# Derek-TH-Wang/OpenRoboRL

Hardware: AMD Instinct MI355X
Metric: env steps/sec at N parallel robots (higher is better)
Workload: dtype f32

## Files before the change

openroborl_amd/csrc/orr_env_kernels.h:

```cpp
#pragma once
#if defined(ORR_PHASE_TIMERS) && !defined(ORR_WAVE_TIMELINE)
#define ORR_WAVE_TIMELINE 1
#endif
#ifndef ORR_TU_MAIN
#undef ORR_PHASE_TIMERS
#endif
#include <hip/hip_runtime.h>
#include <type_traits>
#include <math.h>
#include <stdint.h>
#include <stdio.h>
#include <stdlib.h>
#include <string.h>

#include "orr_device.h"

#ifdef ORR_PHASE_TIMERS
__device__ long long g_phase_cycles[orr::kPhaseSlots];
__device__ long long g_wave_phases[2048 * 40];
#define PT_INIT() do { if (threadIdx.x == 0) { for (int i_ = 0; i_ < orr::kPhaseSlots; i_++) S.pt_acc[i_] = 0; S.pt_last = clock64(); } } while (0)
#define PT(k) do { if (threadIdx.x == 0) { const long long t_ = clock64(); S.pt_acc[k] += t_ - S.pt_last; S.pt_last = clock64(); } } while (0)
#define PT_FLUSH() do { if (threadIdx.x == 0 && blockIdx.x == gridDim.x / 2) for (int i_ = 0; i_ < orr::kPhaseSlots; i_++) atomicAdd((unsigned long long*)&g_phase_cycles[i_], (unsigned long long)S.pt_acc[i_]); \
                        if (threadIdx.x == 0 && blockIdx.x < 2048) for (int i_ = 0; i_ < orr::kPhaseSlots; i_++) g_wave_phases[blockIdx.x * 40 + i_] = S.pt_acc[i_]; } while (0)
#else
// ... 16 lines not shown
#define ORR_DUAL_COUNT(k, cond) do { const unsigned long long b_ = __ballot(cond), act_ = __ballot(1); \
    if (b_ && (int)(threadIdx.x & 63u) == __ffsll((long long)act_) - 1) atomicAdd(&g_dual_contact[k], (unsigned long long)__popcll(b_)); } while (0)
#else
#define ORR_DUAL_COUNT(k, cond)
#endif

using namespace orr;

#define O(name) ORR_OFF_##name

#include "orr_robot_io.h"
#include "orr_physics.h"
#include "orr_task.h"

#define ORR_PROLOGUE()                                                                   \
  __shared__ Shared Sarr[kRPW];                                                          \
  const int wtid = (int)threadIdx.x;                                                     \
  const int wave_id = (int)blockIdx.x;                                                   \
  const int sub = wtid / kLanes, lane = wtid % kLanes;                                   \
  Shared& S = Sarr[sub];                                                                 \
  float* obs = S.ph.end.obs;                                                             \
  const int robot_raw = wave_id * kRPW + sub;                                            \
  const bool in_range = robot_raw < P.cfg.num_robots;                                    \
  const int robot = in_range ? robot_raw : 0;  \
  float* rec = P.state + (size_t)robot * ORR_STATE_STRIDE

template <bool CLIPS = false, bool NOISE = false>
__global__ __launch_bounds__(64) void orr_reset_kernel(KParams P, const uint8_t* mask, float* obs_out, const float* uniforms) {
  ORR_PROLOGUE();
  const bool valid = in_range && !(mask && !mask[robot]);
  load_robot(P, rec, S, lane);
  const long long total = P.counters[ORR_CNT_TOTAL_STEP_COUNT];
  const ResetConst RC = load_reset_const(P, S, lane);
  reset_robot<CLIPS, NOISE>(P, rec, S, lane, valid, total, obs, RC, uniforms ? uniforms + (size_t)robot * 28 : nullptr);
  WSYNC();
  store_robot(rec, S, lane, valid);
  if (valid)
    for (int i = lane; i < ORR_OFFEND_ANCHOR_VALID - ORR_OFF_ANCHOR + 1; i += kLanes) rec[O(ANCHOR) + i] = 0.0f;
  if (obs_out && valid)
    for (int i = lane; i < ORR_OBS_DIM; i += kLanes) obs_out[(size_t)robot * ORR_OBS_DIM + i] = obs[i];
}

#ifndef ORR_WAVES_PER_EU
#define ORR_WAVES_PER_EU 1
#endif
template <int MODE, int WPE = ORR_WAVES_PER_EU, bool ANCHOR = false, bool CLIPS = false, bool NOISE = false>
__global__ __launch_bounds__(64) __attribute__((amdgpu_waves_per_eu(WPE, WPE))) void orr_step_kernel(KParams P, const float* actions, float* obs_out, float* reward_out,
                                                      uint8_t* done_out, int nsub, ReplayArgs RP) {
  constexpr bool TERMS = (MODE & kModeTerms) != 0;
  static_assert(!TERMS || (MODE & 3) != 1, "the debug physics computes no reward");
  constexpr bool CONTACTS = (MODE & kModeContacts) != 0;
  static_assert(!CONTACTS || (MODE & 3) != 2, "the parity replay replaces the physics by recorded states: it has no impulses");
  constexpr bool ACT = (MODE & kModeActuator) != 0;
  static_assert(!ACT || (MODE & 3) != 1, "the debug physics takes its torques as given");
  static_assert(!ACT || TERMS, "the actuator variants are supersets: instantiated with the reward terms only");
  ORR_PROLOGUE();
  const bool valid = in_range;
  const orr_config& c = P.cfg;
  PT_INIT();
  WT_INIT();
  const long long total_snapshot = P.counters[ORR_CNT_TOTAL_STEP_COUNT];
  load_robot(P, rec, S, lane);
  bool terms_bound = true, contacts_bound = true, act_bound = false;
  if constexpr (ACT) {
    terms_bound = P.tab->terms != nullptr;
    contacts_bound = P.tab->contact_out != nullptr;
    act_bound = P.tab->act_out != nullptr;
  }
// ... 186 lines not shown
  bool switched = false;
  if constexpr (CLIPS) {
    if (t >= (double)clip_change) {
      typedef const int __attribute__((address_space(1)))* gip;
      typedef const float __attribute__((address_space(1)))* gfp;
      const int type = geti(S, O(ROBOT_TYPE));
      const int set_n = ((gip)&P.tab->clip_set_n[0])[type];
      const float sw_min = ((gfp)&P.tab->clip_switch[type][0])[0], sw_max = ((gfp)&P.tab->clip_switch[type][0])[1];
      if (set_n > 1 && sw_max < INFINITY) {
        float u4[4];
        philox_block(c.seed, (uint32_t)geti(S, O(ROBOT_INDEX)), (uint32_t)geti(S, O(EPISODE_IDX)), 8u + (uint32_t)geti(S, O(EP_STEP)), u4);
        const uint32_t m = (uint32_t)(u4[0] * 16777216.0f);
        const int k = (int)((m * (uint32_t)set_n) >> 24);
        const int id = ((gip)&P.tab->clip_set[type][0])[k];
        clip_change = clip_change_time(t, sw_min, sw_max, u4[1]);
        WSYNC();
        if (lane == 0) seti(S, O(CLIP_ID), id);
        const unsigned int* cg = reinterpret_cast<const unsigned int*>(&P.tab->clip[id]);
        unsigned int* cl = reinterpret_cast<unsigned int*>(&S.clip);
        if (lane < (int)(sizeof(DevClip) / 4)) cl[lane] = cg[lane];
        WSYNC();
        if (lane == 0) {
          S.s[O(TIME_OFFSET)] = u4[2] * (float)clip.dur_d;
          if (valid) rec[O(CLIP_CHANGE_TIME)] = clip_change;
        }
        WSYNC();
        t = motion_time(P, S);
        switched = true;
      }
    }
  }
  const double step_dt = clip.sim_dt_d * c.action_repeat;
  double tl = t;
  {
    const int k = lane - 1;
    const int steps = (k & 2) ? ((k & 1) ? c.tar_frame_steps[3] : c.tar_frame_steps[2]) : ((k & 1) ? c.tar_frame_steps[1] : c.tar_frame_steps[0]);
    if (lane >= 1 && lane <= 4) tl = t + steps * step_dt;
  }
  PoseLoads PL;
  sample_poses_issue(P, S, lane, tl, PL);
  typedef float __attribute__((address_space(1)))* gterm;
  float term = 0.0f, term_sum = 0.0f;
  if constexpr (TERMS) {
    if (lane < 5 && terms_bound) term_sum = ((gterm)P.tab->term_sums)[(size_t)robot * 5 + lane];
  }
  float c_ep = 0.0f;
  if constexpr (CONTACTS) {
    if (lane < 8 && contacts_bound) c_ep = ((gcontact)P.tab->contact_ep)[(size_t)robot * 8 + lane];
  }
  float a_ep = 0.0f;
  if constexpr (ACT && (MODE & 3) == 0) {
    if (lane < 4 && act_bound) a_ep = ((gact)P.tab->act_ep)[(size_t)robot * 4 + lane];
  }
  float rew;
  if constexpr (TERMS) {
    float tk[5];
    rew = calc_reward<true>(P, S, lane, (MODE & 3) == 2 ? RP.eff + (size_t)robot * 48 : nullptr, tk);
    term = lane == 0 ? tk[0] : (lane == 1 ? tk[1] : (lane == 2 ? tk[2] : (lane == 3 ? tk[3] : tk[4])));
  } else {
    rew = calc_reward(P, S, lane, (MODE & 3) == 2 ? RP.eff + (size_t)robot * 48 : nullptr);
  }
  sample_poses_finish(P, S, lane, tl, true, PL);
  {
    const float ph = clip_phase(clip, t_phase);
    if (lane == 0) {
      bool sync_pos = (c.flags & ORR_FLAG_CYCLE_SYNC) && ph < S.s[O(PREV_PHASE)];
      if constexpr (CLIPS) {
        if (switched) {
          q_about_z(task_heading(S, &S.s[O(QUAT)]) - task_heading(S, &S.ph.end.pose[0][3]), &S.s[O(ORIGIN_ROT)]);
          sync_pos = true;
        }
      }
      if (sync_pos) {
        float pr[3];
        qrot(&S.ph.end.pose[0][0], &S.s[O(ORIGIN_ROT)], pr);
        S.s[O(ORIGIN_POS)] = S.s[O(POS)] - pr[0];
        S.s[O(ORIGIN_POS) + 1] = S.s[O(POS) + 1] - pr[1];
        S.s[O(ORIGIN_POS) + 2] = 0.0f;
      }
      S.s[O(PREV_PHASE)] = ph;
      float v[3];
      qrot(&S.ph.end.vel[0], &S.s[O(ORIGIN_ROT)], v); S.ph.end.vel[0] = v[0]; S.ph.end.vel[1] = v[1]; S.ph.end.vel[2] = v[2];
      qrot(&S.ph.end.vel[3], &S.s[O(ORIGIN_ROT)], v); S.ph.end.vel[3] = v[0]; S.ph.end.vel[4] = v[1]; S.ph.end.vel[5] = v[2];
    }
    WSYNC();
    apply_origin(S, lane, 5);
    for (int i = lane; i < 19; i += kLanes) S.s[O(REF_POSE) + i] = S.ph.end.pose[0][i];
    for (int i = lane; i < 18; i += kLanes) S.s[O(REF_VEL) + i] = S.ph.end.vel[i];
    WSYNC();
  }
  PT(12);
  int reason = 0;
  unsigned long long log_slot = __builtin_nondeterministic_value(log_slot);
  uint32_t noise_i = 0u;
  {
    const float* rp = &S.s[O(REF_POSE)];
    float pe = 0.0f, qc[4], dq[4];
#pragma unroll
    for (int k = 0; k < 3; k++) { float d = rp[k] - S.s[O(POS) + k]; pe += d * d; }
    qconj(&S.s[O(QUAT)], qc);
    qmul(rp + 3, qc, dq);
    const float ang = q_norm_angle(dq);
    if (geti(S, O(STEP_COUNTER)) > 0 && fall) reason |= ORR_DONE_CONTACT_FALL;
    if (pe > c.dist_fail_threshold * c.dist_fail_threshold) reason |= ORR_DONE_ROOT_POS;
    if (fabsf(ang) > c.rot_fail_threshold) reason |= ORR_DONE_ROOT_ROT;
    if (!(clip.flags & ORR_CLIP_WRAP) && t >= clip.dur_d) reason |= ORR_DONE_MOTION_OVER;
    bool bad = false;
    for (int i = lane; i < 37; i += kLanes) bad = bad || !(fabsf(S.s[O(POS) + i]) < 1e30f);
    if (((__ballot(bad) >> (sub * kLanes)) & ((1ull << (kLanes - 1)) * 2ull - 1ull)) != 0ull || S.s[kHead - 1] != 0.0f) reason |= ORR_DONE_NAN;
    if (!(fabsf(rew) < 1e30f)) reason |= ORR_DONE_NAN;
    if (reason & ORR_DONE_NAN) rew = 0.0f;
    const int ep_step = geti(S, O(EP_STEP)) + 1;
    if constexpr (TERMS) {
      if (reason & ORR_DONE_NAN) term = 0.0f;
      term_sum = (ep_step == 1 ? 0.0f : term_sum) + term;
    }
    if constexpr (CONTACTS) {
      if (reason & ORR_DONE_NAN) c_sum = c_max = 0.0f;
      const float nsum = __shfl(c_sum, sub * kLanes + 3 * ((lane & 7) >> 1));
      const float add = nsum > 0.0f ? ((lane & 1) ? nsum : 1.0f) : 0.0f;
      c_ep = (ep_step == 1 ? 0.0f : c_ep) + add;
    }
    if constexpr (ACT) {
      a_w *= c.sim_dt;
      if (reason & ORR_DONE_NAN) a_s1 = a_pk = a_s2 = a_w = 0.0f;
      if constexpr ((MODE & 3) == 0) {
        const bool motor = lane < 12;
        const float w_all = row_sum16(motor ? a_w : 0.0f), s2_all = row_sum16(motor ? a_s2 : 0.0f), pk_all = row_max16(motor ? a_pk : 0.0f);
        const float sat_all = row_max16(motor && !(reason & ORR_DONE_NAN) && a_pk == a_lim ? 1.0f : 0.0f);
        const float old = ep_step == 1 ? 0.0f : a_ep;
        a_ep = lane == 2 ? fmaxf(old, pk_all) : old + (lane == 0 ? w_all : (lane == 1 ? s2_all : sat_all));
      }
    }
    if constexpr (NOISE) noise_i = (uint32_t)ep_step;
    if (ep_step >= geti(S, O(MAX_EP_STEPS))) reason |= ORR_DONE_TIME_LIMIT;
    if (lane == 0 && valid && reason != 0) log_slot = atomicAdd((unsigned long long*)&P.counters[ORR_CNT_EPISODES], 1ull);
    WSYNC();
    if (lane == 0) {
      seti(S, O(EP_STEP), ep_step);
      seti(S, O(DONE_REASON), reason);
      S.s[O(EP_RETURN)] += rew;
    }
  }
  if (lane < 12) obs[lane] = S.s[O(IMU_HIST) + lane];
  for (int i = lane; i < 36; i += kLanes) { obs[12 + i] = S.s[O(LASTACT_HIST) + i]; obs[48 + i] = S.s[O(MOTORANG_HIST) + i]; }
  target_obs<NOISE>(P, rec, S, lane, obs + ORR_PROPRIO_DIM, (uint32_t)geti(S, O(EPISODE_IDX)), noise_i);
  if (valid && lane == 0) {
    reward_out[robot] = rew;
    done_out[robot] = reason != 0;
  }
  if constexpr (TERMS) {
    if (valid && lane < 5 && terms_bound) {
      ((gterm)P.tab->terms)[(size_t)robot * 5 + lane] = term;
      ((gterm)P.tab->term_sums)[(size_t)robot * 5 + lane] = term_sum;
    }
  }
  if constexpr (CONTACTS) {
    store_contacts();
    if (valid && lane < 8 && contacts_bound) ((gcontact)P.tab->contact_ep)[(size_t)robot * 8 + lane] = c_ep;
  }
  if constexpr (ACT) {
    if (valid && lane < 12 && act_bound) {
      typedef f4 __attribute__((address_space(1)))* gact4;
      ((gact4)reinterpret_cast<f4*>(P.tab->act_out))[(size_t)robot * 12 + lane] = f4{a_s1, a_pk, a_s2, a_w};
    }
    if constexpr ((MODE & 3) == 0) {
      if (valid && lane < 4 && act_bound) ((gact)P.tab->act_ep)[(size_t)robot * 4 + lane] = a_ep;
    }
  }
  PT(13);
  if (reason != 0) {
    float log_ret = 0.0f, log_len = 0.0f;
    int log_clip = 0;
    const bool logs = lane == 0 && valid;
    const unsigned long long slot = log_slot;
    if (lane == 0) {
      log_ret = S.s[O(EP_RETURN)]; log_len = (float)geti(S, O(EP_STEP));
      if constexpr (CLIPS) log_clip = geti(S, O(CLIP_ID));
      S.s[O(LAST_EP_RETURN)] = log_ret;
      seti(S, O(LAST_EP_LEN), geti(S, O(EP_STEP)));
    }
    WSYNC();
    if (c.flags & ORR_FLAG_AUTO_RESET) {
      PT(31);
      reset_robot<CLIPS, NOISE>(P, rec, S, lane, valid, total_snapshot, obs, RC);
      if constexpr (ANCHOR) AS = AnchorState{{0.0f, 0.0f, 0.0f}, {0.0f, 0.0f, 0.0f}, 0};
    }
    if (logs && P.ep_log) {
      if (slot < (unsigned long long)P.ep_log_cap) {
        P.ep_log[2 * slot] = log_ret;
        P.ep_log[2 * slot + 1] = log_len;
        if constexpr (CLIPS) {
          int* const clip_log = P.tab->clip_log;
          if (clip_log) clip_log[slot] = log_clip;
        }
      } else {
        atomicAdd((unsigned long long*)&P.counters[ORR_CNT_EPLOG_DROPPED], 1ull);
      }
    }
    if constexpr (TERMS) {
      const int src = sub * kLanes;
      const unsigned long long tslot = ((unsigned long long)(unsigned)__shfl((int)(slot >> 32), src) << 32) | (unsigned)__shfl((int)slot, src);
      gterm const term_log = (gterm)P.tab->term_log;
      if (valid && lane < 5 && P.ep_log && term_log && tslot < (unsigned long long)P.ep_log_cap) term_log[tslot * 5 + lane] = term_sum;
    }
    if constexpr (CONTACTS) {
      const int src = sub * kLanes;
      const unsigned long long cslot = ((unsigned long long)(unsigned)__shfl((int)(slot >> 32), src) << 32) | (unsigned)__shfl((int)slot, src);
      gcontact const contact_log = (gcontact)P.tab->contact_log;
      if (valid && lane < 8 && P.ep_log && contact_log && cslot < (unsigned long long)P.ep_log_cap) contact_log[cslot * 8 + lane] = c_ep;
    }
    if constexpr (ACT && (MODE & 3) == 0) {
      const int src = sub * kLanes;
      const unsigned long long aslot = ((unsigned long long)(unsigned)__shfl((int)(slot >> 32), src) << 32) | (unsigned)__shfl((int)slot, src);
      gact const act_log = (gact)P.tab->act_log;
      if (valid && lane < 4 && P.ep_log && act_log && aslot < (unsigned long long)P.ep_log_cap) act_log[aslot * 4 + lane] = a_ep;
    }
  }
  WSYNC();
  PT(14);
  store_robot(rec, S, lane, valid);
  store_anchor();
  if (valid) {
    typedef f4 __attribute__((address_space(1))) * g4ptr;
    static_assert(ORR_OBS_DIM % 4 == 0, "16-byte pieces");
    const g4ptr od = (g4ptr)reinterpret_cast<f4*>(obs_out + (size_t)robot * ORR_OBS_DIM);
    const f4* os = reinterpret_cast<const f4*>(obs);
#pragma unroll
    for (int k = 0; k < (ORR_OBS_DIM / 4 + kLanes - 1) / kLanes; k++) { const int q = lane + k * kLanes; if (q < ORR_OBS_DIM / 4) od[q] = os[q]; }
  }
  PT(15);
  PT_FLUSH();
  const unsigned long long fin_mask = __ballot(valid && lane == 0 && reason != 0), val_mask = __ballot(valid && lane == 0);
  if (wtid == 0) {
    const unsigned long long add = ((unsigned long long)__popcll(fin_mask) << 32) | (unsigned long long)__popcll(val_mask);
    const unsigned long long now = atomicAdd((unsigned long long*)&P.counters[ORR_CNT_TICKET], add) + add;
    if ((unsigned int)now == (unsigned int)P.cfg.num_robots) {
      atomicAdd((unsigned long long*)&P.counters[ORR_CNT_TOTAL_STEP_COUNT], now >> 32);
      atomicAdd((unsigned long long*)&P.counters[ORR_CNT_TOTAL_TIMESTEPS], (unsigned long long)P.cfg.num_robots);
      atomicExch((unsigned long long*)&P.counters[ORR_CNT_TICKET], 0ull);
    }
  }
  WT_STORE((long long)((fin_mask & 1ull) | ((fin_mask >> 15) & 2ull) | ((fin_mask >> 30) & 4ull) | ((fin_mask >> 45) & 8ull)));
}


#ifdef ORR_STAGE_DUMP
namespace orr {
constexpr int kStageUstar = 0, kStageLc = kStageUstar + 18, kStageLeg = kStageLc + 12 * 18, kStageBf = kStageLeg + 4 * 24;
constexpr int kStageRowWords = 40, kStageRow = kStageBf + kLanes * 27, kStageGeom = kStageRow + kLanes * 2 * kStageRowWords;
constexpr int kStageW = kStageGeom + kLanes * 20, kStageWords = kStageW + kMaxRows * 18;
}
template <bool ANCHOR, int WPE>
__global__ __launch_bounds__(64) __attribute__((amdgpu_waves_per_eu(WPE, WPE))) void orr_stage_dump_kernel(KParams P, const float* torques, float* out, long long out_words) {
  ORR_PROLOGUE();
  (void)obs;
  const bool valid = in_range;
  const orr_config& cfg = P.cfg;
  const long long base = (long long)robot * kStageWords;
  auto put = [&](int k, float v) __attribute__((always_inline)) {
    if (valid && k >= 0 && k < kStageWords && base + k < out_words) out[base + k] = v;
  };
  load_robot(P, rec, S, lane);
  for (int i = lane; i < kMaxRows * kWStride; i += kLanes) (&S.ph.sub.W[0][0])[i] = 0.0f;
  WSYNC();
  LegConst K;
  load_leg_const(P, S, lane, K);
  {
    float rel[4], Rb[9];
// ... 141 lines not shown
```

openroborl_amd/csrc/orr_robot_io.h:

```cpp
#pragma once

typedef float f4 __attribute__((ext_vector_type(4)));
__device__ static void load_robot(const KParams& P, const float* rec, Shared& S, int lane) {
  {
    static_assert(kHead % 4 == 0 && ORR_STATE_STRIDE % 4 == 0, "16-byte pieces");
    typedef const f4 __attribute__((address_space(1))) * g4ptr;
    const g4ptr src = (g4ptr)reinterpret_cast<const f4*>(rec);
    f4* dst = reinterpret_cast<f4*>(S.s);
    constexpr int kQ = kHead / 4, kIt = (kQ + kLanes - 1) / kLanes;
    f4 tmp[kIt];
#pragma unroll
    for (int k = 0; k < kIt; k++) { const int q = lane + k * kLanes; tmp[k] = src[q < kQ ? q : kQ - 1]; }
#pragma unroll
    for (int k = 0; k < kIt; k++) { const int q = lane + k * kLanes; if (q < kQ) dst[q] = tmp[k]; }
  }
  WSYNC();
  const DevModel& gm = P.tab->model[geti(S, O(ROBOT_TYPE))];
  {
    static_assert(sizeof(DevClip) % 4 == 0 && sizeof(DevClip) / 4 <= kLanes, "one word of the clip header per lane");
    const unsigned int* cg = reinterpret_cast<const unsigned int*>(&P.tab->clip[geti(S, O(CLIP_ID))]);
    unsigned int* cl = reinterpret_cast<unsigned int*>(&S.clip);
    if (lane < (int)(sizeof(DevClip) / 4)) cl[lane] = cg[lane];
  }
  {
// ... 32 lines not shown
    int n = (int)(lat / dt);
    if (n + 1 >= len) { k0 = k1 = len - 1; }
    else { k0 = n; k1 = n + 1; al = (lat - n * dt) / dt; }
  }
  const int i0 = (head - k0 + 2 * ORR_RING_DEPTH) % ORR_RING_DEPTH, i1 = (head - k1 + 2 * ORR_RING_DEPTH) % ORR_RING_DEPTH;
  for (int i = lane; i < 19; i += kLanes) {
    float e0 = rec[O(RING) + i0 * ORR_RING_ENTRY + i], e1 = rec[O(RING) + i1 * ORR_RING_ENTRY + i];
    S.co[i] = (k0 == k1) ? e0 : (1.0f - al) * e0 + al * e1;
  }
  WSYNC();
}

__device__ __forceinline__ void base_rotation(Shared& S, int lane, float rel[4], float Rb[9]) {
  float qi[4];
  qinv(S.m.init_quat, qi);
  qmul(&S.s[O(QUAT)], qi, rel);
  q_to_mat(rel, Rb);
#pragma unroll
  for (int i = 0; i < 9; i++) S.Rb[i] = Rb[i];
}

struct ResetConst {
  int j;
  float off, dir;
  float init;
  float p0;
};
__device__ __forceinline__ ResetConst load_reset_const(const KParams& P, const Shared& S, int lane) {
  const ColdPtr mc = model_cold(P, geti(S, O(ROBOT_TYPE)));
  const int ml = lane < 12 ? lane : 0;
  return ResetConst{mc->joint_of_motor[ml], mc->motor_offset[ml], mc->motor_dir[ml], mc->init_motor_angles[ml], mc->init_pos[lane < 3 ? lane : 0]};
}

__device__ static void receive_obs(const KParams& P, float* rec, Shared& S, int lane, bool valid, const ResetConst& RC, float* entry = nullptr) {
  const int head = (geti(S, O(RING_HEAD)) + 1) % ORR_RING_DEPTH, len = geti(S, O(RING_LEN));
  float rel[4], Rb[9], rate[3];
  base_rotation(S, lane, rel, Rb);
  mtv3(Rb, &S.s[O(ANGVEL)], rate);
  for (int i = lane; i < ORR_RING_ENTRY; i += kLanes) {
    float val = 0.0f;
    if (i < 12) {
      static_assert(kLanes >= 12, "the first pass of the loop covers the twelve motors");
      val = (S.s[O(Q) + RC.j] - RC.off) * RC.dir;
    } else if (i < 16) {
      val = i == 12 ? rel[0] : (i == 13 ? rel[1] : (i == 14 ? rel[2] : rel[3]));
    } else if (i < 19) {
      val = i == 16 ? rate[0] : (i == 17 ? rate[1] : rate[2]);
    }
    if (valid) rec[O(RING) + head * ORR_RING_ENTRY + i] = val;
    if (entry) entry[i] = val;
  }
  WSYNC();
  if (lane == 0) {
    seti(S, O(RING_HEAD), head);
    seti(S, O(RING_LEN), len + 1 > ORR_RING_DEPTH ? ORR_RING_DEPTH : len + 1);
  }
  WSYNC();
}

struct RingFetch {
  float e0[2], e1[2];
  float al;
  bool new0, new1, same;
};
struct RingLatency {
  int n;
  float al;
  bool none;
};
__device__ __forceinline__ RingLatency ring_latency(const KParams& P, const Shared& S) {
  const float lat = S.s[O(LATENCY)], dt = P.cfg.sim_dt;
  RingLatency L;
  L.none = lat <= 0.0f;
  L.n = (int)(lat / dt);
  L.al = (lat - L.n * dt) / dt;
  return L;
}
struct RingCursor { int head, len; };
__device__ __forceinline__ int ring_wrap_up(int i) { return i >= ORR_RING_DEPTH ? i - ORR_RING_DEPTH : i; }
__device__ __forceinline__ int ring_wrap_down(int i) { return i < 0 ? i + ORR_RING_DEPTH : i; }
__device__ __forceinline__ void ring_prefetch(const RingLatency& L, const float* rec, const RingCursor& C, int lane, RingFetch& F) {
  const int head = ring_wrap_up(C.head + 1);
  const int len = C.len + 1 > ORR_RING_DEPTH ? ORR_RING_DEPTH : C.len + 1;
  int k0 = 0, k1 = 0;
  F.al = 0.0f;
  if (!(L.none || len == 1)) {
    if (L.n + 1 >= len) { k0 = k1 = len - 1; }
    else { k0 = L.n; k1 = L.n + 1; F.al = L.al; }
  }
  F.same = k0 == k1; F.new0 = k0 == 0; F.new1 = k1 == 0;
// ... 31 lines not shown
```

openroborl_amd/csrc/orr_task.h:

```cpp
#pragma once

struct Sample {
  int f0, f1, count;
  float blend, phase;
};
__device__ __forceinline__ double clip_phase_d(const DevClip& c, double t) {
  double ph = t / c.dur_d;
  if (c.flags & ORR_CLIP_WRAP) ph -= floor(ph);
  else ph = fmin(fmax(ph, 0.0), 1.0);
  return ph;
}
__device__ __forceinline__ float clip_phase(const DevClip& c, double t) { return (float)clip_phase_d(c, t); }
__device__ __forceinline__ Sample clip_index(const DevClip& c, double t) {
  Sample s;
  const bool wrap = c.flags & ORR_CLIP_WRAP;
  s.count = (int)floor(t / c.dur_d);
  if (!wrap) s.count = s.count < 0 ? 0 : (s.count > 1 ? 1 : s.count);
  const double ph = clip_phase_d(c, t);
  s.phase = (float)ph;
  if (!wrap && t <= 0.0) { s.f0 = 0; s.f1 = 0; s.blend = 0.0f; }
  else if (!wrap && t >= c.dur_d) { s.f0 = c.F - 1; s.f1 = c.F - 1; s.blend = 0.0f; }
  else {
    s.f0 = (int)(ph * (c.F - 1));
    s.f0 = s.f0 > c.F - 1 ? c.F - 1 : s.f0;
// ... 110 lines not shown
        for (int k = 0; k < 18; k++) S.ph.end.vel[k] = 0.0f;
      } else {
        float v[18], cp[3], cr[4], t3[3];
#pragma unroll
        for (int k = 0; k < 18; k++) v[k] = (1.0f - sm.blend) * S.ph.end.fvel[0][k] + sm.blend * S.ph.end.fvel[1][k];
        cycle_offset(c, sm.count, cp, cr);
        qrot(&v[0], cr, t3); v[0] = t3[0]; v[1] = t3[1]; v[2] = t3[2];
        qrot(&v[3], cr, t3); v[3] = t3[0]; v[4] = t3[1]; v[5] = t3[2];
#pragma unroll
        for (int k = 0; k < 18; k++) S.ph.end.vel[k] = v[k];
      }
    }
  }
  WSYNC();
}

__device__ static void apply_origin(Shared& S, int lane, int nt) {
  if (lane < nt) {
    float qq[4], pp[3];
    qmul(&S.s[O(ORIGIN_ROT)], &S.ph.end.pose[lane][3], qq);
    qrot(&S.ph.end.pose[lane][0], &S.s[O(ORIGIN_ROT)], pp);
    S.ph.end.pose[lane][0] = pp[0] + S.s[O(ORIGIN_POS)]; S.ph.end.pose[lane][1] = pp[1] + S.s[O(ORIGIN_POS) + 1]; S.ph.end.pose[lane][2] = pp[2] + S.s[O(ORIGIN_POS) + 2];
    S.ph.end.pose[lane][3] = qq[0]; S.ph.end.pose[lane][4] = qq[1]; S.ph.end.pose[lane][5] = qq[2]; S.ph.end.pose[lane][6] = qq[3];
  }
  WSYNC();
}

__device__ __forceinline__ double motion_time(const KParams& P, const Shared& S) {
  double t = geti(S, O(STATE_ACTION_COUNTER)) * S.clip.sim_dt_d + (double)S.s[O(TIME_OFFSET)];
  if (geti(S, O(WARMUP))) t -= (double)P.cfg.warmup_time;
  return t;
}

constexpr uint32_t kNoiseResetBlock = 0x20000000u, kNoiseHeadingBlock = 0x30000000u;

template <bool NOISE = false>
__device__ static void target_obs(const KParams& P, const float* rec, Shared& S, int lane, float* obs76, uint32_t episode = 0u, uint32_t noise_i = 0u) {
  if (lane >= 1 && lane <= 4) {
    float rpy[3];
    euler_from_quat(&S.co[12], rpy);
    float sy, cy, spch, cpch;
    joint_sincos(rpy[1], &spch, &cpch);
    joint_sincos(rpy[2], &sy, &cy);
    float heading = atan2_bf(sy * cpch, cy * cpch);
    if constexpr (NOISE) {
      typedef const float __attribute__((address_space(1)))* gfp;
      const float sigma = ((gfp)&P.tab->noise.tar_heading_std)[0];
      float u4[4], z0, z1;
      philox_block(P.cfg.seed, (uint32_t)geti(S, O(ROBOT_INDEX)), episode, kNoiseHeadingBlock + noise_i, u4);
      normal_pair(u4[0], u4[1], &z0, &z1);
      heading = fmaf(sigma, z0, heading);
    }
    float ih[4], p[3], pr[3], q[4];
    q_about_z(-heading, ih);
    const float* pose = S.ph.end.pose[lane];
    p[0] = pose[0] - S.s[O(REF_POSE)]; p[1] = pose[1] - S.s[O(REF_POSE) + 1]; p[2] = pose[2] - S.s[O(REF_POSE) + 2];
    qrot(p, ih, pr);
    qmul(ih, pose + 3, q);
    qstd(q);
    float* o = obs76 + (lane - 1) * 19;
    o[0] = pr[0]; o[1] = pr[1]; o[2] = pr[2]; o[3] = q[0]; o[4] = q[1]; o[5] = q[2]; o[6] = q[3];
#pragma unroll
    for (int k = 7; k < 19; k++) o[k] = pose[k];
  }
  WSYNC();
}
// ... 126 lines not shown
  double t = (double)total / (double)c.curriculum_steps;
  t = t < 0.0 ? 0.0 : (t > 1.0 ? 1.0 : t);
  t = t * t * t;
  return (int)((1.0 - t) * c.ep_len_start + t * c.ep_len_end);
}

__device__ static void sensors_push(Shared& S, int lane, bool fill_all) {
  float rpy[3];
  euler_from_quat(&S.co[12], rpy);
  constexpr int kCols = (28 + kLanes - 1) / kLanes;
  float newest[kCols], h0[kCols], h1[kCols];
  int base[kCols], w[kCols], kk[kCols];
#pragma unroll
  for (int c = 0; c < kCols; c++) {
    const int col = lane + c * kLanes;
    base[c] = 0; w[c] = 0; kk[c] = 0; newest[c] = 0.0f; h0[c] = 0.0f; h1[c] = 0.0f;
    if (col < 12) { base[c] = O(MOTORANG_HIST); w[c] = 12; kk[c] = col; newest[c] = map_pi(S.co[col]); }
    else if (col < 16) { base[c] = O(IMU_HIST); w[c] = 4; kk[c] = col - 12; newest[c] = kk[c] == 0 ? rpy[0] : (kk[c] == 1 ? rpy[1] : (kk[c] == 2 ? S.co[16] : S.co[17])); }
    else if (col < 28) { base[c] = O(LASTACT_HIST); w[c] = 12; kk[c] = col - 16; newest[c] = S.s[O(LAST_ACTION) + kk[c]]; }
    if (col < 28) { h0[c] = S.s[base[c] + kk[c]]; h1[c] = S.s[base[c] + w[c] + kk[c]]; }
  }
  WSYNC();
#pragma unroll
  for (int c = 0; c < kCols; c++) {
    if (lane + c * kLanes < 28) {
      S.s[base[c] + kk[c]] = newest[c];
      S.s[base[c] + w[c] + kk[c]] = fill_all ? newest[c] : h0[c];
      S.s[base[c] + 2 * w[c] + kk[c]] = fill_all ? newest[c] : h1[c];
    }
  }
  WSYNC();
}

template <bool CLIPS = false, bool NOISE = false>
__device__ static void reset_robot(const KParams& P, float* rec, Shared& S, int lane, bool valid, long long total_step_count, float* obs,
                                   const ResetConst& RC, const float* uni_replay = nullptr) {
  const orr_config& c = P.cfg;
  const uint32_t robot = (uint32_t)geti(S, O(ROBOT_INDEX)), ep = (uint32_t)geti(S, O(EPISODE_IDX)) + 1u;
  WSYNC();
  if (lane == 0) seti(S, O(EPISODE_IDX), (int)ep);
  const int rj = RC.j;
  const float r_q0 = RC.init + RC.off, r_p0 = RC.p0;
  if (lane < 3) {
    S.s[O(POS) + lane] = r_p0 + (lane < 2 ? S.s[O(GRID_OFFSET) + lane] : 0.0f);
    S.s[O(LINVEL) + lane] = 0.0f; S.s[O(ANGVEL) + lane] = 0.0f;
  }
  if (lane < 4) S.s[O(QUAT) + lane] = S.m.init_quat[lane];
  if (lane < 12) {
    const int j = rj;
    S.s[O(Q) + j] = r_q0;
    S.s[O(QD) + j] = 0.0f;
    S.s[O(LAST_ACTION) + lane] = 0.0f; S.s[O(ACTION) + lane] = 0.0f; S.s[O(FILTER_ACTION) + lane] = 0.0f; S.s[O(LAMBDA) + lane] = 0.0f;
    S.s[O(XHIST) + lane] = 0.0f; S.s[O(XHIST) + 12 + lane] = 0.0f; S.s[O(YHIST) + lane] = 0.0f; S.s[O(YHIST) + 12 + lane] = 0.0f;
  }
  if (lane == 0) {
    seti(S, O(RING_LEN), 0); seti(S, O(RING_HEAD), ORR_RING_DEPTH - 1);
    seti(S, O(STATE_ACTION_COUNTER), 0); seti(S, O(STEP_COUNTER), 0); seti(S, O(FILTER_VALID), 0);
    seti(S, O(EP_STEP), 0);
    S.s[O(EP_RETURN)] = 0.0f;
  }
  WSYNC();
  PT(16);
  float* draws = S.ph.end.red + 24;
  static_assert(kLanes == 16, "reset_robot / the pose sampler assume 16 lanes per robot");
  int set_id = 0, set_n = 0;
  float sw_min = 0.0f, sw_max = 0.0f;
  if constexpr (CLIPS) {
    static_assert(ORR_MAX_CLIPS == kLanes, "one clip-set entry per lane");
    typedef const int __attribute__((address_space(1)))* gip;
    typedef const float __attribute__((address_space(1)))* gfp;
    const int type = geti(S, O(ROBOT_TYPE));
    set_id = ((gip)&P.tab->clip_set[type][0])[lane];
    set_n = ((gip)&P.tab->clip_set_n[0])[type];
    sw_min = ((gfp)&P.tab->clip_switch[type][0])[0];
    sw_max = ((gfp)&P.tab->clip_switch[type][0])[1];
  }
  if (lane < (CLIPS ? 8 : 7)) {
    float u4[4];
    if (uni_replay && (!CLIPS || lane < 7)) { u4[0] = uni_replay[4 * lane]; u4[1] = uni_replay[4 * lane + 1]; u4[2] = uni_replay[4 * lane + 2]; u4[3] = uni_replay[4 * lane + 3]; }
    else philox_block(c.seed, robot, ep, (uint32_t)lane, u4);
    draws[4 * lane] = u4[0]; draws[4 * lane + 1] = u4[1]; draws[4 * lane + 2] = u4[2]; draws[4 * lane + 3] = u4[3];
  }
  WSYNC();
  float u_change = 0.0f;
  if constexpr (CLIPS) {
    u_change = draws[29];
    const uint32_t m = (uint32_t)(draws[28] * 16777216.0f);
    const int k = (int)((m * (uint32_t)set_n) >> 24);
    if (set_n > 0 && lane == k) seti(S, O(CLIP_ID), set_id);
    WSYNC();
    const unsigned int* cg = reinterpret_cast<const unsigned int*>(&P.tab->clip[geti(S, O(CLIP_ID))]);
    unsigned int* cl = reinterpret_cast<unsigned int*>(&S.clip);
    if (lane < (int)(sizeof(DevClip) / 4)) cl[lane] = cg[lane];
    WSYNC();
  }
  float* nz = &S.ph.end.ee[0][0][0];
  float n_prob = 0.0f, n_pos = 0.0f, n_rot = 0.0f, n_jp = 0.0f, n_vel = 0.0f, n_ang = 0.0f, n_jv = 0.0f;
// ... 1 lines not shown
    static_assert(sizeof(S.ph.end.ee) >= 36 * sizeof(float), "U(0..3) + 32 normals");
    typedef const float __attribute__((address_space(1)))* gfp;
    const gfp ns = (gfp)&P.tab->noise.perturb_init_state_prob;
    n_prob = ns[0]; n_pos = ns[1]; n_rot = ns[2]; n_jp = ns[3]; n_vel = ns[4]; n_ang = ns[5]; n_jv = ns[6];
    if (lane < 9) {
      float u4[4];
      philox_block(c.seed, robot, ep, kNoiseResetBlock + (uint32_t)lane, u4);
      nz[4 * lane] = u4[0]; nz[4 * lane + 1] = u4[1]; nz[4 * lane + 2] = u4[2]; nz[4 * lane + 3] = u4[3];
    }
    WSYNC();
    float z0, z1;
    normal_pair(nz[4 + 2 * lane], nz[5 + 2 * lane], &z0, &z1);
    WSYNC();
    nz[4 + 2 * lane] = z0; nz[5 + 2 * lane] = z1;
    WSYNC();
  }
  PT(24);
  const DevClip& clip = S.clip;
  {
    const float u1 = draws[26], u2 = draws[27];
    const bool ref_init = u1 < c.ref_state_init_prob;
    const bool warm = (!ref_init) && c.warmup_time > 0.0f;
    if (lane == 0) {
      seti(S, O(WARMUP), warm ? 1 : 0);
      S.s[O(TIME_OFFSET)] = warm ? u2 * c.warmup_time : u2 * (float)clip.dur_d;
      S.s[O(ORIGIN_POS)] = 0.0f; S.s[O(ORIGIN_POS) + 1] = 0.0f; S.s[O(ORIGIN_POS) + 2] = 0.0f;
      S.s[O(ORIGIN_ROT)] = 0.0f; S.s[O(ORIGIN_ROT) + 1] = 0.0f; S.s[O(ORIGIN_ROT) + 2] = 0.0f; S.s[O(ORIGIN_ROT) + 3] = 1.0f;
    }
    WSYNC();
  }
  const double t = motion_time(P, S);
  const double step_dt = S.clip.sim_dt_d * c.action_repeat;
  double tl = t;
  {
    const int k = lane - 1;
    const int steps = (k & 2) ? ((k & 1) ? c.tar_frame_steps[3] : c.tar_frame_steps[2]) : ((k & 1) ? c.tar_frame_steps[1] : c.tar_frame_steps[0]);
    if (lane >= 1 && lane <= 4) tl = t + steps * step_dt;
  }
  PT(20);
  PoseLoads PL;
  sample_poses_issue(P, S, lane, tl, PL, 26);
  PT(19);
  float* e1 = S.ph.end.red;
  receive_obs(P, rec, S, lane, valid, RC, e1);
  PT(17);
  WSYNC();
  for (int i = lane; i < 19; i += kLanes) S.co[i] = e1[i];
  WSYNC();
  PT(29);
  sensors_push(S, lane, true);
  const float e1_keep[2] = {e1[lane], e1[lane < 3 ? 16 + lane : lane]};
  PT(18);
  if (c.flags & ORR_FLAG_RANDOMIZER) {
    for (int i = lane; i < 26; i += kLanes) {
      const float u = draws[i];
      if (i < 2) S.s[O(INERTIA_RATIO) + i] = 0.5f + u * 1.0f;
      else if (i < 10) { if (((i - 2) & 1) == 0) S.s[O(KNEE_FRICTION) + ((i - 2) >> 1)] = u * 0.05f; }
      else if (i == 10) S.s[O(LATENCY)] = u * 0.04f;
      else if (i == 11) S.s[O(FOOT_MU)] = 0.5f + u * 0.75f;
      else if (i < 14) S.s[O(MASS_RATIO) + i - 12] = 0.8f + u * 0.4f;
      else S.s[O(STRENGTH) + i - 14] = 0.8f + u * 0.4f;
    }
    WSYNC();
  }
  PT(25);
  sample_poses_finish(P, S, lane, tl, true, PL, 26);
  PT(21);
  if (lane == 0) {
    S.s[O(ORIGIN_POS)] = S.s[O(POS)] - S.ph.end.pose[0][0];
    S.s[O(ORIGIN_POS) + 1] = S.s[O(POS) + 1] - S.ph.end.pose[0][1];
    S.s[O(ORIGIN_POS) + 2] = 0.0f;
    const float dh = qheading(&S.s[O(QUAT)]) - qheading(&S.ph.end.pose[0][3]);
    q_about_z(dh, &S.s[O(ORIGIN_ROT)]);
    S.s[O(PREV_PHASE)] = clip_phase(clip, t);
    if constexpr (CLIPS) { if (valid) rec[O(CLIP_CHANGE_TIME)] = clip_change_time(t, sw_min, sw_max, u_change); }
  }
  WSYNC();
  apply_origin(S, lane, 5);
  for (int i = lane; i < 19; i += kLanes) S.s[O(REF_POSE) + i] = S.ph.end.pose[0][i];
  if (lane == 0) {
    float v[3];
    qrot(&S.ph.end.vel[0], &S.s[O(ORIGIN_ROT)], v); S.ph.end.vel[0] = v[0]; S.ph.end.vel[1] = v[1]; S.ph.end.vel[2] = v[2];
    qrot(&S.ph.end.vel[3], &S.s[O(ORIGIN_ROT)], v); S.ph.end.vel[3] = v[0]; S.ph.end.vel[4] = v[1]; S.ph.end.vel[5] = v[2];
  }
  WSYNC();
  for (int i = lane; i < 18; i += kLanes) S.s[O(REF_VEL) + i] = S.ph.end.vel[i];
  if (lane < 3) { S.s[O(POS) + lane] = S.ph.end.pose[0][lane]; S.s[O(LINVEL) + lane] = S.ph.end.vel[lane]; S.s[O(ANGVEL) + lane] = S.ph.end.vel[3 + lane]; }
  if (lane < 4) S.s[O(QUAT) + lane] = S.ph.end.pose[0][3 + lane];
  if (lane < 12) { S.s[O(Q) + lane] = S.ph.end.pose[0][7 + lane]; S.s[O(QD) + lane] = S.ph.end.vel[6 + lane]; }
  if constexpr (NOISE) {
    if (nz[0] < n_prob) {
      const float* z = nz + 4;
      if (lane < 2) { S.s[O(POS) + lane] = fmaf(n_pos, z[lane], S.ph.end.pose[0][lane]); S.s[O(LINVEL) + lane] = fmaf(n_vel, z[15 + lane], S.ph.end.vel[lane]); }
      if (lane < 3) S.s[O(ANGVEL) + lane] = fmaf(n_ang, z[17 + lane], S.ph.end.vel[3 + lane]);
      if (lane < 12) { S.s[O(Q) + lane] = fmaf(n_jp, z[3 + lane], S.ph.end.pose[0][7 + lane]); S.s[O(QD) + lane] = fmaf(n_jv, z[20 + lane], S.ph.end.vel[6 + lane]); }
      const float a0 = fmaf(2.0f, nz[1], -1.0f), a1 = fmaf(2.0f, nz[2], -1.0f), a2 = fmaf(2.0f, nz[3], -1.0f);
      const float n2 = a0 * a0 + a1 * a1 + a2 * a2;
      float sh, ch;
      joint_sincos(0.5f * (n_rot * z[2]), &sh, &ch);
      const float ax = n2 < 1e-30f ? 0.0f : sh * rsq(n2);
      const float dq[4] = {a0 * ax, a1 * ax, a2 * ax, n2 < 1e-30f ? 1.0f : ch};
      float qp[4];
      qmul(dq, &S.ph.end.pose[0][3], qp);
      if (lane < 4) S.s[O(QUAT) + lane] = pick4(lane, qp[0], qp[1], qp[2], qp[3]);
    }
  }
  WSYNC();
  PT(22);
  float* e2 = S.ph.end.red + 56;
  receive_obs(P, rec, S, lane, valid, RC, e2);
  {
    const float lat = S.s[O(LATENCY)], dt = c.sim_dt;
    const int n = (int)(lat / dt);
    const float al = (lat - n * dt) / dt;
    WSYNC();
    for (int i = lane; i < 19; i += kLanes) {
      const float newest = e2[i], oldest = i < 16 ? e1_keep[0] : e1_keep[1];
      S.co[i] = lat <= 0.0f ? newest : (n + 1 >= 2 ? oldest : (1.0f - al) * newest + al * oldest);
    }
    WSYNC();
  }
  if (lane == 0) seti(S, O(MAX_EP_STEPS), time_limit(c, total_step_count));
  if (lane < 12) obs[lane] = S.s[O(IMU_HIST) + lane];
  for (int i = lane; i < 36; i += kLanes) { obs[12 + i] = S.s[O(LASTACT_HIST) + i]; obs[48 + i] = S.s[O(MOTORANG_HIST) + i]; }
  PT(23);
  target_obs<NOISE>(P, rec, S, lane, obs + ORR_PROPRIO_DIM, ep, 0u);
  PT(30);
}
```

Measured before the change: 21.76 million.

## Defer reset global stores and build observation once after auto-reset

Reset is split into a state-only reset and a separate observation builder. In the step kernel the observation is built once, after any auto-reset, instead of being built and then rebuilt when the robot resets. Ring-entry and clip-change global writes during reset are collected and written in one batch at the end. The episode-counter and ticket atomics are issued together so their latency overlaps, and the frame-step lookup is pinned to scalar registers. This trades some reordering complexity and extra live state (clip_change, was_reset) for fewer redundant observation builds and scattered global stores on reset paths.

```diff
diff --git a/openroborl_amd/csrc/orr_env_kernels.h b/openroborl_amd/csrc/orr_env_kernels.h
--- a/openroborl_amd/csrc/orr_env_kernels.h
+++ b/openroborl_amd/csrc/orr_env_kernels.h
@@ -72,8 +72,11 @@
   load_robot(P, rec, S, lane);
   const long long total = P.counters[ORR_CNT_TOTAL_STEP_COUNT];
   const ResetConst RC = load_reset_const(P, S, lane);
-  reset_robot<CLIPS, NOISE>(P, rec, S, lane, valid, total, obs, RC, uniforms ? uniforms + (size_t)robot * 28 : nullptr);
-  WSYNC();
+  float clip_change = 0.0f;
+  const uint32_t ep = reset_robot_state<CLIPS, NOISE>(P, S, lane, total, RC, &clip_change, uniforms ? uniforms + (size_t)robot * 28 : nullptr);
+  build_obs<NOISE>(P, rec, S, lane, obs, ep, 0u);
+  WSYNC();
+  store_reset_extras<CLIPS>(rec, S, lane, valid, clip_change);
   store_robot(rec, S, lane, valid);
   if (valid)
     for (int i = lane; i < ORR_OFFEND_ANCHOR_VALID - ORR_OFF_ANCHOR + 1; i += kLanes) rec[O(ANCHOR) + i] = 0.0f;
@@ -326,11 +329,7 @@
   }
   const double step_dt = clip.sim_dt_d * c.action_repeat;
   double tl = t;
-  {
-    const int k = lane - 1;
-    const int steps = (k & 2) ? ((k & 1) ? c.tar_frame_steps[3] : c.tar_frame_steps[2]) : ((k & 1) ? c.tar_frame_steps[1] : c.tar_frame_steps[0]);
-    if (lane >= 1 && lane <= 4) tl = t + steps * step_dt;
-  }
+  if (lane >= 1 && lane <= 4) tl = t + target_frame_steps(c, lane) * step_dt;
   PoseLoads PL;
   sample_poses_issue(P, S, lane, tl, PL);
   typedef float __attribute__((address_space(1)))* gterm;
@@ -385,7 +384,6 @@
   }
   PT(12);
   int reason = 0;
-  unsigned long long log_slot = __builtin_nondeterministic_value(log_slot);
   uint32_t noise_i = 0u;
   {
     const float* rp = &S.s[O(REF_POSE)];
@@ -428,7 +426,6 @@
     }
     if constexpr (NOISE) noise_i = (uint32_t)ep_step;
     if (ep_step >= geti(S, O(MAX_EP_STEPS))) reason |= ORR_DONE_TIME_LIMIT;
-    if (lane == 0 && valid && reason != 0) log_slot = atomicAdd((unsigned long long*)&P.counters[ORR_CNT_EPISODES], 1ull);
     WSYNC();
     if (lane == 0) {
       seti(S, O(EP_STEP), ep_step);
@@ -436,38 +433,12 @@
       S.s[O(EP_RETURN)] += rew;
     }
   }
-  if (lane < 12) obs[lane] = S.s[O(IMU_HIST) + lane];
-  for (int i = lane; i < 36; i += kLanes) { obs[12 + i] = S.s[O(LASTACT_HIST) + i]; obs[48 + i] = S.s[O(MOTORANG_HIST) + i]; }
-  target_obs<NOISE>(P, rec, S, lane, obs + ORR_PROPRIO_DIM, (uint32_t)geti(S, O(EPISODE_IDX)), noise_i);
-  if (valid && lane == 0) {
-    reward_out[robot] = rew;
-    done_out[robot] = reason != 0;
-  }
-  if constexpr (TERMS) {
-    if (valid && lane < 5 && terms_bound) {
-      ((gterm)P.tab->terms)[(size_t)robot * 5 + lane] = term;
-      ((gterm)P.tab->term_sums)[(size_t)robot * 5 + lane] = term_sum;
-    }
-  }
-  if constexpr (CONTACTS) {
-    store_contacts();
-    if (valid && lane < 8 && contacts_bound) ((gcontact)P.tab->contact_ep)[(size_t)robot * 8 + lane] = c_ep;
-  }
-  if constexpr (ACT) {
-    if (valid && lane < 12 && act_bound) {
-      typedef f4 __attribute__((address_space(1)))* gact4;
-      ((gact4)reinterpret_cast<f4*>(P.tab->act_out))[(size_t)robot * 12 + lane] = f4{a_s1, a_pk, a_s2, a_w};
-    }
-    if constexpr ((MODE & 3) == 0) {
-      if (valid && lane < 4 && act_bound) ((gact)P.tab->act_ep)[(size_t)robot * 4 + lane] = a_ep;
-    }
-  }
   PT(13);
+  float log_ret = 0.0f, log_len = 0.0f;
+  int log_clip = 0;
+  uint32_t obs_episode = (uint32_t)geti(S, O(EPISODE_IDX));
+  bool was_reset = false;
   if (reason != 0) {
-    float log_ret = 0.0f, log_len = 0.0f;
-    int log_clip = 0;
-    const bool logs = lane == 0 && valid;
-    const unsigned long long slot = log_slot;
     if (lane == 0) {
       log_ret = S.s[O(EP_RETURN)]; log_len = (float)geti(S, O(EP_STEP));
       if constexpr (CLIPS) log_clip = geti(S, O(CLIP_ID));
@@ -477,9 +448,62 @@
     WSYNC();
     if (c.flags & ORR_FLAG_AUTO_RESET) {
       PT(31);
-      reset_robot<CLIPS, NOISE>(P, rec, S, lane, valid, total_snapshot, obs, RC);
+      obs_episode = reset_robot_state<CLIPS, NOISE>(P, S, lane, total_snapshot, RC, &clip_change);
+      noise_i = 0u;
+      was_reset = true;
       if constexpr (ANCHOR) AS = AnchorState{{0.0f, 0.0f, 0.0f}, {0.0f, 0.0f, 0.0f}, 0};
     }
+  }
+  WSYNC();
+  PT(14);
+  build_obs<NOISE>(P, rec, S, lane, obs, obs_episode, noise_i);
+  PT(13);
+  if (valid && lane == 0) {
+    reward_out[robot] = rew;
+    done_out[robot] = reason != 0;
+  }
+  if constexpr (TERMS) {
+    if (valid && lane < 5 && terms_bound) {
+      ((gterm)P.tab->terms)[(size_t)robot * 5 + lane] = term;
+      ((gterm)P.tab->term_sums)[(size_t)robot * 5 + lane] = term_sum;
+    }
+  }
+  if constexpr (CONTACTS) {
+    store_contacts();
+    if (valid && lane < 8 && contacts_bound) ((gcontact)P.tab->contact_ep)[(size_t)robot * 8 + lane] = c_ep;
+  }
+  if constexpr (ACT) {
+    if (valid && lane < 12 && act_bound) {
+      typedef f4 __attribute__((address_space(1)))* gact4;
+      ((gact4)reinterpret_cast<f4*>(P.tab->act_out))[(size_t)robot * 12 + lane] = f4{a_s1, a_pk, a_s2, a_w};
+    }
+    if constexpr ((MODE & 3) == 0) {
+      if (valid && lane < 4 && act_bound) ((gact)P.tab->act_ep)[(size_t)robot * 4 + lane] = a_ep;
+    }
+  }
+  if (was_reset) store_reset_extras<CLIPS>(rec, S, lane, valid, clip_change);
+  store_robot(rec, S, lane, valid);
+  store_anchor();
+  if (valid) {
+    typedef f4 __attribute__((address_space(1))) * g4ptr;
+    static_assert(ORR_OBS_DIM % 4 == 0, "16-byte pieces");
+    const g4ptr od = (g4ptr)reinterpret_cast<f4*>(obs_out + (size_t)robot * ORR_OBS_DIM);
+    const f4* os = reinterpret_cast<const f4*>(obs);
+#pragma unroll
+    for (int k = 0; k < (ORR_OBS_DIM / 4 + kLanes - 1) / kLanes; k++) { const int q = lane + k * kLanes; if (q < ORR_OBS_DIM / 4) od[q] = os[q]; }
+  }
+  PT(15);
+  PT_FLUSH();
+  const unsigned long long fin_mask = __ballot(valid && lane == 0 && reason != 0), val_mask = __ballot(valid && lane == 0);
+  const unsigned long long add = ((unsigned long long)__popcll(fin_mask) << 32) | (unsigned long long)__popcll(val_mask);
+  unsigned long long log_slot = __builtin_nondeterministic_value(log_slot), ticket = __builtin_nondeterministic_value(ticket);
+  if (lane == 0 && valid && reason != 0) log_slot = atomicAdd((unsigned long long*)&P.counters[ORR_CNT_EPISODES], 1ull);
+  const int tally_lane = WPE == 2 ? (int)__lane_id() : wtid;
+  if (tally_lane == 0) ticket = atomicAdd((unsigned long long*)&P.counters[ORR_CNT_TICKET], add);
+  asm volatile("" : "+v"(log_slot), "+v"(ticket));
+  if (reason != 0) {
+    const bool logs = lane == 0 && valid;
+    const unsigned long long slot = log_slot;
     if (logs && P.ep_log) {
       if (slot < (unsigned long long)P.ep_log_cap) {
         P.ep_log[2 * slot] = log_ret;
@@ -511,24 +535,8 @@
       if (valid && lane < 4 && P.ep_log && act_log && aslot < (unsigned long long)P.ep_log_cap) act_log[aslot * 4 + lane] = a_ep;
     }
   }
-  WSYNC();
-  PT(14);
-  store_robot(rec, S, lane, valid);
-  store_anchor();
-  if (valid) {
-    typedef f4 __attribute__((address_space(1))) * g4ptr;
-    static_assert(ORR_OBS_DIM % 4 == 0, "16-byte pieces");
-    const g4ptr od = (g4ptr)reinterpret_cast<f4*>(obs_out + (size_t)robot * ORR_OBS_DIM);
-    const f4* os = reinterpret_cast<const f4*>(obs);
-#pragma unroll
-    for (int k = 0; k < (ORR_OBS_DIM / 4 + kLanes - 1) / kLanes; k++) { const int q = lane + k * kLanes; if (q < ORR_OBS_DIM / 4) od[q] = os[q]; }
-  }
-  PT(15);
-  PT_FLUSH();
-  const unsigned long long fin_mask = __ballot(valid && lane == 0 && reason != 0), val_mask = __ballot(valid && lane == 0);
-  if (wtid == 0) {
-    const unsigned long long add = ((unsigned long long)__popcll(fin_mask) << 32) | (unsigned long long)__popcll(val_mask);
-    const unsigned long long now = atomicAdd((unsigned long long*)&P.counters[ORR_CNT_TICKET], add) + add;
+  if (tally_lane == 0) {
+    const unsigned long long now = ticket + add;
     if ((unsigned int)now == (unsigned int)P.cfg.num_robots) {
       atomicAdd((unsigned long long*)&P.counters[ORR_CNT_TOTAL_STEP_COUNT], now >> 32);
       atomicAdd((unsigned long long*)&P.counters[ORR_CNT_TOTAL_TIMESTEPS], (unsigned long long)P.cfg.num_robots);
diff --git a/openroborl_amd/csrc/orr_robot_io.h b/openroborl_amd/csrc/orr_robot_io.h
--- a/openroborl_amd/csrc/orr_robot_io.h
+++ b/openroborl_amd/csrc/orr_robot_io.h
@@ -88,7 +88,7 @@
   return ResetConst{mc->joint_of_motor[ml], mc->motor_offset[ml], mc->motor_dir[ml], mc->init_motor_angles[ml], mc->init_pos[lane < 3 ? lane : 0]};
 }
 
-__device__ static void receive_obs(const KParams& P, float* rec, Shared& S, int lane, bool valid, const ResetConst& RC, float* entry = nullptr) {
+__device__ static void receive_obs(Shared& S, int lane, const ResetConst& RC, float* entry) {
   const int head = (geti(S, O(RING_HEAD)) + 1) % ORR_RING_DEPTH, len = geti(S, O(RING_LEN));
   float rel[4], Rb[9], rate[3];
   base_rotation(S, lane, rel, Rb);
@@ -103,8 +103,7 @@
     } else if (i < 19) {
       val = i == 16 ? rate[0] : (i == 17 ? rate[1] : rate[2]);
     }
-    if (valid) rec[O(RING) + head * ORR_RING_ENTRY + i] = val;
-    if (entry) entry[i] = val;
+    entry[i] = val;
   }
   WSYNC();
   if (lane == 0) {
@@ -112,6 +111,14 @@
     seti(S, O(RING_LEN), len + 1 > ORR_RING_DEPTH ? ORR_RING_DEPTH : len + 1);
   }
   WSYNC();
+}
+__device__ __forceinline__ void store_ring_entry(float* rec, int lane, bool valid, int head, const float* entry) {
+  static_assert(ORR_RING_ENTRY == 20 && kLanes == 16, "lane mapping of an entry's words");
+  if (valid) {
+    float* dst = rec + O(RING) + head * ORR_RING_ENTRY;
+    dst[lane] = entry[lane];
+    if (lane < 4) dst[16 + lane] = entry[16 + lane];
+  }
 }
 
 struct RingFetch {
diff --git a/openroborl_amd/csrc/orr_task.h b/openroborl_amd/csrc/orr_task.h
--- a/openroborl_amd/csrc/orr_task.h
+++ b/openroborl_amd/csrc/orr_task.h
@@ -166,6 +166,15 @@
   return t;
 }
 
+__device__ __forceinline__ int target_frame_steps(const orr_config& c, int lane) {
+  int i0 = 0;
+  asm("" : "+s"(i0));
+  int s0 = c.tar_frame_steps[i0], s1 = c.tar_frame_steps[i0 + 1], s2 = c.tar_frame_steps[i0 + 2], s3 = c.tar_frame_steps[i0 + 3];
+  asm("" : "+s"(s0), "+s"(s1), "+s"(s2), "+s"(s3));
+  const int k = lane - 1;
+  return (k & 2) ? ((k & 1) ? s3 : s2) : ((k & 1) ? s1 : s0);
+}
+
 constexpr uint32_t kNoiseResetBlock = 0x20000000u, kNoiseHeadingBlock = 0x30000000u;
 
 template <bool NOISE = false>
@@ -358,37 +367,21 @@
   WSYNC();
 }
 
+__device__ __forceinline__ float* reset_entry1(Shared& S) { return S.ph.end.red; }
+__device__ __forceinline__ float* reset_entry2(Shared& S) { return S.ph.end.red + 56; }
 template <bool CLIPS = false, bool NOISE = false>
-__device__ static void reset_robot(const KParams& P, float* rec, Shared& S, int lane, bool valid, long long total_step_count, float* obs,
-                                   const ResetConst& RC, const float* uni_replay = nullptr) {
+__device__ static uint32_t reset_robot_state(const KParams& P, Shared& S, int lane, long long total_step_count, const ResetConst& RC,
+                                             float* clip_change, const float* uni_replay = nullptr) {
   const orr_config& c = P.cfg;
   const uint32_t robot = (uint32_t)geti(S, O(ROBOT_INDEX)), ep = (uint32_t)geti(S, O(EPISODE_IDX)) + 1u;
   WSYNC();
-  if (lane == 0) seti(S, O(EPISODE_IDX), (int)ep);
-  const int rj = RC.j;
-  const float r_q0 = RC.init + RC.off, r_p0 = RC.p0;
-  if (lane < 3) {
-    S.s[O(POS) + lane] = r_p0 + (lane < 2 ? S.s[O(GRID_OFFSET) + lane] : 0.0f);
-    S.s[O(LINVEL) + lane] = 0.0f; S.s[O(ANGVEL) + lane] = 0.0f;
-  }
-  if (lane < 4) S.s[O(QUAT) + lane] = S.m.init_quat[lane];
-  if (lane < 12) {
-    const int j = rj;
-    S.s[O(Q) + j] = r_q0;
-    S.s[O(QD) + j] = 0.0f;
-    S.s[O(LAST_ACTION) + lane] = 0.0f; S.s[O(ACTION) + lane] = 0.0f; S.s[O(FILTER_ACTION) + lane] = 0.0f; S.s[O(LAMBDA) + lane] = 0.0f;
-    S.s[O(XHIST) + lane] = 0.0f; S.s[O(XHIST) + 12 + lane] = 0.0f; S.s[O(YHIST) + lane] = 0.0f; S.s[O(YHIST) + 12 + lane] = 0.0f;
-  }
   if (lane == 0) {
-    seti(S, O(RING_LEN), 0); seti(S, O(RING_HEAD), ORR_RING_DEPTH - 1);
-    seti(S, O(STATE_ACTION_COUNTER), 0); seti(S, O(STEP_COUNTER), 0); seti(S, O(FILTER_VALID), 0);
-    seti(S, O(EP_STEP), 0);
-    S.s[O(EP_RETURN)] = 0.0f;
-  }
-  WSYNC();
+    seti(S, O(EPISODE_IDX), (int)ep);
+    seti(S, O(STATE_ACTION_COUNTER), 0);
+  }
   PT(16);
   float* draws = S.ph.end.red + 24;
-  static_assert(kLanes == 16, "reset_robot / the pose sampler assume 16 lanes per robot");
+  static_assert(kLanes == 16, "reset_robot_state / the pose sampler assume 16 lanes per robot");
   int set_id = 0, set_n = 0;
   float sw_min = 0.0f, sw_max = 0.0f;
   if constexpr (CLIPS) {
@@ -456,17 +449,34 @@
   const double t = motion_time(P, S);
   const double step_dt = S.clip.sim_dt_d * c.action_repeat;
   double tl = t;
-  {
-    const int k = lane - 1;
-    const int steps = (k & 2) ? ((k & 1) ? c.tar_frame_steps[3] : c.tar_frame_steps[2]) : ((k & 1) ? c.tar_frame_steps[1] : c.tar_frame_steps[0]);
-    if (lane >= 1 && lane <= 4) tl = t + steps * step_dt;
-  }
+  if (lane >= 1 && lane <= 4) tl = t + target_frame_steps(c, lane) * step_dt;
   PT(20);
   PoseLoads PL;
   sample_poses_issue(P, S, lane, tl, PL, 26);
   PT(19);
-  float* e1 = S.ph.end.red;
-  receive_obs(P, rec, S, lane, valid, RC, e1);
+  const int rj = RC.j;
+  const float r_q0 = RC.init + RC.off, r_p0 = RC.p0;
+  if (lane < 3) {
+    S.s[O(POS) + lane] = r_p0 + (lane < 2 ? S.s[O(GRID_OFFSET) + lane] : 0.0f);
+    S.s[O(LINVEL) + lane] = 0.0f; S.s[O(ANGVEL) + lane] = 0.0f;
+  }
+  if (lane < 4) S.s[O(QUAT) + lane] = S.m.init_quat[lane];
+  if (lane < 12) {
+    const int j = rj;
+    S.s[O(Q) + j] = r_q0;
+    S.s[O(QD) + j] = 0.0f;
+    S.s[O(LAST_ACTION) + lane] = 0.0f; S.s[O(ACTION) + lane] = 0.0f; S.s[O(FILTER_ACTION) + lane] = 0.0f; S.s[O(LAMBDA) + lane] = 0.0f;
+    S.s[O(XHIST) + lane] = 0.0f; S.s[O(XHIST) + 12 + lane] = 0.0f; S.s[O(YHIST) + lane] = 0.0f; S.s[O(YHIST) + 12 + lane] = 0.0f;
+  }
+  if (lane == 0) {
+    seti(S, O(RING_LEN), 0); seti(S, O(RING_HEAD), ORR_RING_DEPTH - 1);
+    seti(S, O(STEP_COUNTER), 0); seti(S, O(FILTER_VALID), 0);
+    seti(S, O(EP_STEP), 0);
+    S.s[O(EP_RETURN)] = 0.0f;
+  }
+  WSYNC();
+  float* e1 = reset_entry1(S);
+  receive_obs(S, lane, RC, e1);
   PT(17);
   WSYNC();
   for (int i = lane; i < 19; i += kLanes) S.co[i] = e1[i];
@@ -497,8 +507,8 @@
     const float dh = qheading(&S.s[O(QUAT)]) - qheading(&S.ph.end.pose[0][3]);
     q_about_z(dh, &S.s[O(ORIGIN_ROT)]);
     S.s[O(PREV_PHASE)] = clip_phase(clip, t);
-    if constexpr (CLIPS) { if (valid) rec[O(CLIP_CHANGE_TIME)] = clip_change_time(t, sw_min, sw_max, u_change); }
-  }
+  }
+  if constexpr (CLIPS) *clip_change = clip_change_time(t, sw_min, sw_max, u_change);
   WSYNC();
   apply_origin(S, lane, 5);
   for (int i = lane; i < 19; i += kLanes) S.s[O(REF_POSE) + i] = S.ph.end.pose[0][i];
@@ -531,8 +541,8 @@
   }
   WSYNC();
   PT(22);
-  float* e2 = S.ph.end.red + 56;
-  receive_obs(P, rec, S, lane, valid, RC, e2);
+  float* e2 = reset_entry2(S);
+  receive_obs(S, lane, RC, e2);
   {
     const float lat = S.s[O(LATENCY)], dt = c.sim_dt;
     const int n = (int)(lat / dt);
@@ -545,9 +555,20 @@
     WSYNC();
   }
   if (lane == 0) seti(S, O(MAX_EP_STEPS), time_limit(c, total_step_count));
+  PT(23);
+  return ep;
+}
+
+template <bool CLIPS = false>
+__device__ __forceinline__ void store_reset_extras(float* rec, Shared& S, int lane, bool valid, float clip_change) {
+  store_ring_entry(rec, lane, valid, 0, reset_entry1(S));
+  store_ring_entry(rec, lane, valid, 1, reset_entry2(S));
+  if constexpr (CLIPS) { if (valid && lane == 0) rec[O(CLIP_CHANGE_TIME)] = clip_change; }
+}
+
+template <bool NOISE = false>
+__device__ static void build_obs(const KParams& P, const float* rec, Shared& S, int lane, float* obs, uint32_t episode, uint32_t noise_i) {
   if (lane < 12) obs[lane] = S.s[O(IMU_HIST) + lane];
   for (int i = lane; i < 36; i += kLanes) { obs[12 + i] = S.s[O(LASTACT_HIST) + i]; obs[48 + i] = S.s[O(MOTORANG_HIST) + i]; }
-  PT(23);
-  target_obs<NOISE>(P, rec, S, lane, obs + ORR_PROPRIO_DIM, ep, 0u);
-  PT(30);
-}
+  target_obs<NOISE>(P, rec, S, lane, obs + ORR_PROPRIO_DIM, episode, noise_i);
+}
```

Measured after the change: 22.22 million (median of 6 runs). 1.02x the previous value.
